# kskjs1203/SevenNet_finetuning

Measured on AMD Instinct MI355X. Metric: atoms/sec energy+force, SevenNet-0 lmax=2, 97,336-atom box @1 GPU, higher is better.
Workload: dtype f32 (MLP / linear products on bf16 MFMA pieces: bf16x6 fwd, bf16x3 bwd); 1 GPU; SevenNet-0 energy+force+virial, 97,336-atom periodic Si box (23^3 cells), 1 GPU; total_atoms=97336, scaling=weak, atoms_per_rank=97336, edges_per_rank=2725408, parallelism=single

## Files before the change

sevennet_finetuning_amd/csrc/api.cpp:

```cpp
#include <hip/hip_runtime.h>

#include <algorithm>
#include <cstdio>
#include <cstdlib>
#include <cstring>
#include <string>
#include <vector>

#include "../../include/e3gnn.h"
#include "api_util.h"
#include "atom_virial.h"
#include "cg_tables.h"
#include "common.h"
#include "dbuf.h"
#include "fused.h"
#include "generic.h"
#include "model.h"
#include "node.h"
#include "tp.h"

using namespace e3gnn;

namespace {
thread_local std::string g_err;
// ... 643 lines not shown
    const FcnDims& fd = m->fcnd;
    double flops = 2.0 * nl * dl, bytes = nl * 4.0 * (dl + 2);
    if (m->fcn) {
      double mac = fd.w[fd.nh];
      for (int k = 0; k < fd.nh; ++k) mac += (double)fd.w[k] * fd.w[k + 1];
      flops = 4.0 * nl * mac;
      bytes = nl * 4.0 * (2 * dl + 2);
    }
    Region r(c, s, C_READOUT, flops, bytes);
    if (m->fcn)
      HIPCHK(launch_readout_fcn((int)nl, fd, c->x[L].f(), m->fcn_w.f(), c->type.i(), m->scale.f(),
                                m->shift.f(), c->eat.f(), c->grad[L].f(), s));
    else
      HIPCHK(launch_readout((int)nl, dl, c->x[L].f(), m->readout_v.f(), c->type.i(), m->scale.f(),
                            m->shift.f(), c->eat.f(), s));
    HIPCHK(launch_sum(nl, c->eat.f(), c->part.f(), energy ? energy : c->scratch6.f(), s));
    if (atomic_energy && nl > 0)
      HIPCHK(hipMemcpyAsync(atomic_energy, c->eat.p, nl * 4, hipMemcpyDeviceToDevice, s));
    if (!m->fcn)
      HIPCHK(launch_readout_bwd((int)nl, dl, m->readout_v.f(), c->type.i(), m->scale.f(),
                                c->grad[L].f(), s));
  }
  c->readout_done = 1;
  return E3GNN_OK;
}

static int v1_conv_backward(e3gnn_ctx* c, int t, hipStream_t s) {
  e3gnn_model* m = c->m;
  const int64_t nl = c->nl, E = c->E;
  const int dx = irreps_dim(m->irreps[t]), dm = irreps_dim(m->mid[t]), W = m->W[t];
  const int kind = t == 0 ? 0 : (t == m->nlayer - 1 ? 2 : 1);
  {
    Region r(c, s, C_TP_BWD, 3.0 * tp_flops_per_edge(m->kcode(t)) * E,
             (double)E * 4 * (2 * W + 2 * 9 + dx + (t > 0 ? dx : 0) + 2) + nl * 4.0 * dm);
    TpArgs a;
    std::memset(&a, 0, sizeof(a));
    a.row_ptr = c->row_ptr.i();
    a.nbr = c->nbr.i();
    a.Y = c->Y.f();
    a.w = c->w[t].f();
    a.h = c->h[t].f();
    a.gagg = c->agg.f();
    a.dw = c->dw.f();
    a.dxc = t > 0 ? c->dxc.f() : nullptr;
    a.dYacc = c->dY.f();
    a.n_centers = (int)nl;
    HIPCHK(launch_tp_bwd(kind, a, s));
  }
  {
    Region r(c, s, C_MLP_BWD, 2.0 * E * (64 * W + 64 * 64 + 64 * 8),
             (double)E * 4 * (W + 64 * 6 + 16));
    auto& mm = m->mlp[t];
    GemmBatch b;
    std::memset(&b, 0, sizeof(b));
    GemmProb p = base_prob();
    p.A = c->dw.f(); p.lda = W; p.K = W;
    p.B = mm.w2t.f(); p.ldb = 64; p.N = 64;
    p.C = c->H2.f(); p.ldc = 64; p.M = (int)E;
    p.act = 2; p.pre_in = c->a2[t].f();
    add_prob(b, p);
    HIPCHK(launch_gemm(b, s));
    std::memset(&b, 0, sizeof(b));
    p.A = c->H2.f(); p.lda = 64; p.K = 64;
    p.B = mm.w1t.f(); p.C = c->H1.f(); p.pre_in = c->a1[t].f();
    add_prob(b, p);
    HIPCHK(launch_gemm(b, s));
    std::memset(&b, 0, sizeof(b));
    p.A = c->H1.f(); p.B = mm.w0t.f(); p.ldb = 8; p.N = 8;
    p.C = c->demb.f(); p.ldc = 8; p.act = 0; p.pre_in = nullptr; p.beta = 1;
    add_prob(b, p);
    HIPCHK(launch_gemm(b, s));
  }
  return E3GNN_OK;
}

int e3gnn_layer_backward_part(e3gnn_ctx* c, int t, int part, void* stream) {
  if (!c) return fail(E3GNN_ERR_ARG, "null context");
  e3gnn_model* m = c->m;
  if (t < 0 || t >= m->nlayer) return fail(E3GNN_ERR_ARG, "layer out of range");
  if (part != 0 && part != 1) return fail(E3GNN_ERR_ARG, "part must be 0 or 1");
  if (!c->readout_done) return fail(E3GNN_ERR_ARG, "e3gnn_readout must precede the backward");
  HIPCHK(hipSetDevice(m->device));
  hipStream_t s = (hipStream_t)stream;
  if (c->gen) {
    if (part == 0) HIPCHK(gen_layer_backward(c->gen, m->gen, gen_graph(c), t, s));
    return E3GNN_OK;
  }
  const int64_t n = c->n, nl = c->nl, E = c->E;
  const int dx = irreps_dim(m->irreps[t]), dg = irreps_dim(m->gin[t]);
  const int dm = irreps_dim(m->mid[t]), W = m->W[t];
  const bool last = t == m->nlayer - 1;
  const int kind = t == 0 ? 0 : (last ? 2 : 1);
  const int code = m->kcode(t);
  const int64_t n_int = c->n_int, e_int = c->e_int;
  auto out_bwd = [&]() -> int {
    {
      Region r(c, s, C_GATE_BWD, 0, nl * 4.0 * (2 * dg + irreps_dim(m->irreps[t + 1])));
      HIPCHK(launch_gate_bwd((int)nl, last, m->gdims[t], c->y[t].f(), c->grad[t + 1].f(), c->dy.f(), s));
    }
    Region r(c, s, C_LINEAR, lin_flops(*m->si2[t], nl));
    NlBatch nb;
    if (c->nodelin && nl_batch(nb, *m->nl_si2t[t], c->dy.f(), dg, nullptr, 0, c->agg.f(), dm, nl, 0))
      HIPCHK(launch_nodelin(nb, s));
    else
      HIPCHK(launch_gemm(lin_bwd(*m->si2[t], c->dy.f(), dg, c->agg.f(), dm, nl, 0), s));
    return E3GNN_OK;
  };
  auto in_bwd = [&](int64_t r0, int64_t r1, bool gather, bool owned) -> int {
    if (t == 0) return E3GNN_OK;
    if (gather && r1 > r0) {
      Region r(c, s, C_GATHER, 0, (double)E * 4 * (dx + 1) * (r1 - r0) / std::max<int64_t>(n, 1) +
                                      (r1 - r0) * 4.0 * dx);
      HIPCHK(launch_gather_rows_range((int)r0, (int)r1, dx, c->src_ptr.i(), c->src_perm.i(),
                                      c->dxc.f(), c->dh.f(), s));
    }
    Region r(c, s, C_LINEAR, lin_flops(*m->si1[t], r1 - r0) + (owned ? lin_flops(*m->sc[t], nl) : 0));
    NlBatch b0, b1;
    const int64_t p1 = owned ? nl : r0;
    if (c->nodelin && (!owned || r0 == 0) && r1 >= p1 &&
        (!owned || nl_batch(b0, *m->nl_bwd[t], c->dh.f(), dx, c->dy.f(), dg, c->grad[t].f(), dx, nl, 0)) &&
        (r1 == p1 || nl_batch(b1, *m->nl_si1t[t], c->dh.f() + p1 * dx, dx, nullptr, 0,
                              c->grad[t].f() + p1 * dx, dx, r1 - p1, 0))) {
      if (owned) HIPCHK(launch_nodelin(b0, s));
      if (r1 > p1) HIPCHK(launch_nodelin(b1, s));
    } else {
      if (r1 > r0)
        HIPCHK(launch_gemm(lin_bwd(*m->si1[t], c->dh.f() + r0 * dx, dx, c->grad[t].f() + r0 * dx, dx,
                                   r1 - r0, 0), s));
      if (owned) HIPCHK(launch_gemm(lin_bwd(*m->sc[t], c->dy.f(), dg, c->grad[t].f(), dx, nl, 1), s));
    }
    return E3GNN_OK;
  };
  if (c->graph_impl == 1) {
    if (part == 1) return E3GNN_OK;
    if (const int rc = out_bwd()) return rc;
    if (const int rc = v1_conv_backward(c, t, s)) return rc;
    return in_bwd(0, n, true, true);
  }
  if (part == 0) {
    if (const int rc = out_bwd()) return rc;
  }
  FusedArgs a = fused_base(c, t);
  a.gagg = c->agg.f();
  a.center = c->center.i();
  a.n_edges = (int)E;
  a.src_ptr = c->src_ptr.i();
  a.src_perm = c->src_perm.i();
  a.dh = c->dh.f();
  a.dxc = (!last && t > 0) ? c->dxc.f() : nullptr;
  a.dgu = c->dgu.f();
  a.demb = c->demb.f();
  a.c_begin = (int)(part == 0 ? n_int : 0);
  a.c_end = (int)(part == 0 ? nl : n_int);
  a.node_begin = (int)(part == 0 ? nl : 0);
  a.node_end = (int)(part == 0 ? n : nl);
  double ef = (double)(part == 0 ? E - e_int : e_int);
  if (last && c->timing && a.node_end > a.node_begin) {
    int32_t q[2];
    HIPCHK(hipMemcpyAsync(&q[0], a.src_ptr + a.node_begin, 4, hipMemcpyDeviceToHost, s));
    HIPCHK(hipMemcpyAsync(&q[1], a.src_ptr + a.node_end, 4, hipMemcpyDeviceToHost, s));
    HIPCHK(hipStreamSynchronize(s));
    ef = (double)(q[1] - q[0]);
  }
  if (last ? a.node_end > a.node_begin : a.c_end > a.c_begin) {
    const double xf = 3.0 * tp_flops_per_edge(code) + 2.0 * (64 * W + 64 * 64 + 8 * 64);
    Region r(c, s, C_CONV_BWD_X + kind, xf * ef,
             ef * 4 * (8 + 9 + 2 + 3 + 8) + (a.c_end - a.c_begin) * 4.0 * dm);
    HIPCHK(last ? launch_conv_bwd_nbr_last(code, a, s) : launch_conv_bwd_ls(code, a, s));
  }
  return part == 0 ? in_bwd(nl, n, !last, false) : in_bwd(0, nl, !last, true);
}

int e3gnn_layer_backward(e3gnn_ctx* c, int t, void* stream) {
  const int rc = e3gnn_layer_backward_part(c, t, 0, stream);
  return rc ? rc : e3gnn_layer_backward_part(c, t, 1, stream);
}

int e3gnn_forces(e3gnn_ctx* c, float* forces, float* virial6, float* edge_grad, void* stream) {
  if (!c) return fail(E3GNN_ERR_ARG, "null context");
  e3gnn_model* m = c->m;
  HIPCHK(hipSetDevice(m->device));
  hipStream_t s = (hipStream_t)stream;
  if (c->gen) {
    HIPCHK(gen_forces(c->gen, m->gen, gen_graph(c), forces, virial6, edge_grad, s));
    c->forces_done = 1;
    return E3GNN_OK;
  }
  const int64_t n = c->n, nl = c->nl, E = c->E;
  {
    Region r(c, s, C_EDGE_FORCE, 0, (double)E * 4 * (3 + 9 + 8 + 3));
    HIPCHK(launch_edge_force(E, c->vec.f(), m->coeffs.f(), m->cutoff, m->r_on, m->raw_sh, c->dY.f(),
                             c->dgu.f(), c->demb.f(), c->fe.f(), c->vpart.f(), s));
    HIPCHK(launch_final_sum(edge_force_blocks(E), 6, c->vpart.f(),
                            virial6 ? virial6 : c->scratch6.f(), s));
  }
  if (forces) {
    Region r(c, s, C_ATOM_FORCE, 0, (double)E * 4 * 2 * 4 + n * 12.0);
    HIPCHK(launch_atom_force((int)n, (int)nl, c->row_ptr.i(), c->src_ptr.i(), c->src_perm.i(),
                             c->fe.f(), forces, s));
  }
  if (edge_grad && E > 0)
    HIPCHK(hipMemcpyAsync(edge_grad, c->fe.p, E * 12, hipMemcpyDeviceToDevice, s));
  c->forces_done = 1;
  return E3GNN_OK;
}

int e3gnn_atom_virial(e3gnn_ctx* c, float* atom_virial6, void* stream) {
  if (!c) return fail(E3GNN_ERR_ARG, "null context");
  if (!atom_virial6) return fail(E3GNN_ERR_ARG, "null atom_virial6 output");
  if (!c->forces_done)
    return fail(E3GNN_ERR_ARG, "e3gnn_forces (or e3gnn_energy_forces) on the current graph must "
                               "precede e3gnn_atom_virial");
  HIPCHK(hipSetDevice(c->m->device));
  hipStream_t s = (hipStream_t)stream;
  const bool ordered = c->done_pending;
  if (ordered && c->done_stream != s) HIPCHK(hipStreamWaitEvent(s, c->done_ev, 0));
  const float* fe = c->gen ? gen_fe(c->gen) : c->fe.f();
  {
    Region r(c, s, C_ATOM_VIRIAL, 18.0 * 2 * c->E, (double)c->E * 4 * 2 * 7 + c->n * 24.0);
    HIPCHK(launch_atom_virial((int)c->n, (int)c->nl, c->row_ptr.i(), c->src_ptr.i(),
                              c->src_perm.i(), c->vec.f(), fe, atom_virial6, s));
  }
  if (ordered) {
    HIPCHK(hipEventRecord(c->done_ev, s));
    c->done_stream = s;
  }
  return E3GNN_OK;
}

int e3gnn_energy_forces(e3gnn_ctx* c, int64_t n_atoms, int64_t n_edges, const int32_t* type,
                        const int32_t* edge_center, const int32_t* edge_nbr,
                        const float* edge_vec, float* energy, float* atomic_energy,
                        float* forces, float* virial6, float* edge_grad, void* stream) {
  if (!energy) return fail(E3GNN_ERR_ARG, "energy output is required");
  int rc = e3gnn_graph_set(c, n_atoms, 0, n_edges, type, edge_center, edge_nbr, edge_vec, stream);
  if (rc) return rc;
  const int L = c->m->nlayer;
  for (int t = 0; t < L; ++t)
    if ((rc = e3gnn_layer_forward(c, t, stream))) return rc;
  if ((rc = e3gnn_readout(c, energy, atomic_energy, stream))) return rc;
  for (int t = L - 1; t >= 0; --t)
    if ((rc = e3gnn_layer_backward(c, t, stream))) return rc;
  if ((rc = e3gnn_forces(c, forces, virial6, edge_grad, stream))) return rc;
  if (!c->stream_ordered) {
    HIPCHK(hipStreamSynchronize((hipStream_t)stream));
  } else {
    if (!c->done_ev) HIPCHK(hipEventCreateWithFlags(&c->done_ev, hipEventDisableTiming));
    HIPCHK(hipEventRecord(c->done_ev, (hipStream_t)stream));
    c->done_stream = (hipStream_t)stream;
    c->done_pending = true;
  }
  return E3GNN_OK;
}

int e3gnn_halo_pack(const int32_t* idx, int64_t n, int dim, const float* src, int64_t src_stride,
                    float* dst, void* stream) {
  if (n < 0 || dim <= 0) return fail(E3GNN_ERR_ARG, "bad halo size");
  HIPCHK(launch_pack(n, dim, idx, src, src_stride, dst, (hipStream_t)stream));
  return E3GNN_OK;
}
int e3gnn_halo_unpack(const int32_t* idx, int64_t n, int dim, const float* src, float* dst,
                      int64_t dst_stride, int accumulate, void* stream) {
  if (n < 0 || dim <= 0) return fail(E3GNN_ERR_ARG, "bad halo size");
  HIPCHK(launch_unpack(n, dim, idx, src, dst, dst_stride, accumulate, (hipStream_t)stream));
  return E3GNN_OK;
}

int e3gnn_set_interior(e3gnn_ctx* c, int64_t n_interior) {
  if (!c) return fail(E3GNN_ERR_ARG, "null context");
  if (n_interior < 0) return fail(E3GNN_ERR_ARG, "negative n_interior");
  c->n_interior_req = n_interior;
  return E3GNN_OK;
}

int e3gnn_set_impl(e3gnn_ctx* c, int impl) {
  if (!c) return fail(E3GNN_ERR_ARG, "null context");
  if (impl != 0 && impl != 1) return fail(E3GNN_ERR_ARG, "impl must be 0 (fused) or 1 (v1)");
  c->impl = impl;
  return E3GNN_OK;
}

int e3gnn_set_timing(e3gnn_ctx* c, int enable) {
  if (!c) return fail(E3GNN_ERR_ARG, "null context");
  c->flush();
  c->timing = enable != 0;
  return E3GNN_OK;
}
int e3gnn_set_stream_ordered(e3gnn_ctx* c, int enable) {
  if (!c) return fail(E3GNN_ERR_ARG, "null context");
  c->stream_ordered = enable != 0;
  return E3GNN_OK;
}
int e3gnn_kernel_stats(e3gnn_ctx* c, const char** names, double* ms, int64_t* launches,
                       double* flops, double* bytes, int max) {
  if (!c) return -1;
  c->flush();
  for (int i = 0; i < C_NCLS && i < max; ++i) {
    if (names) names[i] = kClassNames[i];
    if (ms) ms[i] = c->stats[i].ms;
    if (launches) launches[i] = c->stats[i].launches;
    if (flops) flops[i] = c->stats[i].flops;
    if (bytes) bytes[i] = c->stats[i].bytes;
  }
  return C_NCLS;
}
int e3gnn_reset_stats(e3gnn_ctx* c) {
// ... 59 lines not shown
```

sevennet_finetuning_amd/csrc/fused.h:

```cpp
#pragma once
#include <hip/hip_runtime.h>
#include <cstdint>

namespace e3gnn {

struct MlpW {
  const float* w0;
  const float* w2r;
  const uint16_t* w2b;
  const uint16_t* w2d;
  const uint16_t* w2v;
  const uint16_t* w2s;
  const uint16_t* w1b;
  const uint16_t* w1tb;
  const uint16_t* w0tb;
};

struct FusedArgs {
  const int* row_ptr;
  const int* center;
  const int* nbr;
  const float* emb;
  const float* Y;
  const float* h;
  float* agg;
  const float* gagg;
  const int* src_ptr;
  const int* src_perm;
  float* dh;
  float* dxc;
  float* dgu;
  float* demb;
  MlpW W;
  int n_centers;
  int n_edges;
  int n_nodes;
  float denom;
  int c_begin, c_end, node_begin, node_end;
};

hipError_t launch_conv_fwd(int kind, const FusedArgs& a, hipStream_t s);
hipError_t launch_conv_bwd_ls(int kind, const FusedArgs& a, hipStream_t s);
hipError_t launch_conv_bwd_nbr_last(int kind, const FusedArgs& a, hipStream_t s);

}
```

sevennet_finetuning_amd/csrc/fused.hip:

```cpp
#include "cg_tables.h"
#include "common.h"
#include "fused.h"
#include "tp.h"
#include "w2_image.h"

#include <type_traits>


namespace e3gnn {
namespace {

typedef float f32x4 __attribute__((ext_vector_type(4)));

template <int N, int I = 0, class F>
constexpr void sfor_host(F&& f) {
  if constexpr (I < N) {
    f(std::integral_constant<int, I>{});
    sfor_host<N, I + 1>(f);
  }
}
template <int N, int I = 0, class F>
__device__ __forceinline__ void sfor(F&& f) {
  if constexpr (I < N) {
    f(std::integral_constant<int, I>{});
// ... 887 lines not shown
                wnxt[0] = w2_block_bwd<false>(hq[0], wq);
                wnxt[1] = two ? w2_block_bwd<false>(hq[1], wq) : zero4();
              }
              if (nb + 2 < NBLK) load_w2b(wq, R.w2v, lane, 16 * (nb + 2));
              float dwr2[2][4];
#pragma unroll
              for (int u = 0; u < 2; ++u) {
                if (u == 1 && !two) break;
                float dwr[4];
#pragma unroll
                for (int r = 0; r < 4; ++r) {
                  phase();
                  float dy[2 * p.l2 + 1];
#pragma unroll
                  for (int q = 0; q < 2 * p.l2 + 1; ++q) dy[q] = 0.f;
                  dwr[r] = tp_bwd_xw<p.l1, p.l2, p.l3>(x + r * D1, y[u] + yoff(p.l2), wv[u][r], gm[u] + r * D3,
                                                       dx + r * D1, dy);
                  if constexpr (p.l2 > 0) {
#pragma unroll
                    for (int q = 0; q < 2 * p.l2 + 1; ++q) dYa[u][yoff(p.l2) + q] += dy[q];
                  }
                  pin<D1>(dx + r * D1);
                  pin<8>(dYa[u] + 1);
                }
                if constexpr (NBR_DH2_BF16) {
#pragma unroll
                  for (int r = 0; r < 4; ++r) dwr2[u][r] = u == 1 && !two ? 0.f : dwr[r];
                } else {
#pragma unroll
                  for (int bh = 0; bh < 4; ++bh)
#pragma unroll
                    for (int r = 0; r < 4; ++r) dh2[u][bh] = mfma(bq[bh][r], dwr[r], dh2[u][bh]);
                }
              }
              if constexpr (NBR_DH2_BF16) {
                if (!two) {
#pragma unroll
                  for (int r = 0; r < 4; ++r) dwr2[1][r] = 0.f;
                }
                if (nb & 1) {
                  dh2_pair_g2(dh2, dwp, dwr2, two, R.w2d, nb >> 1, lane);
                } else {
#pragma unroll
                  for (int u = 0; u < 2; ++u)
#pragma unroll
                    for (int r = 0; r < 4; ++r) dwp[u][r] = dwr2[u][r];
                }
              }
              pin<4 * D1>(dx);
              wcur[0] = wnxt[0];
              wcur[1] = wnxt[1];
              ++nb;
            }
          });
          phase();
          {
            constexpr int NV = 4 * D1;
            static_assert(NV % 8 == 4, "batches of 16, 8, then 4");
            float* da = dacc + XOFF + (16 * jj + 4 * g) * D1;
            if constexpr (NV >= 16) da[own] += row_scatter16<16>(dx, rsel);
            if constexpr (NV % 16 >= 8) da[NV / 16 * 16 + (own & 7)] += row_scatter16<8>(dx + NV / 16 * 16, rsel);
            da[NV / 8 * 8 + (own & 3)] += row_scatter16<4>(dx + NV / 8 * 8, rsel);
          }
        }
      }
    });

#pragma unroll
    for (int u = 0; u < 2; ++u) {
      if (u == 1 && !two) break;
      phase();
      float d[8];
#pragma unroll
      for (int q = 0; q < 8; ++q) d[q] = sum_rows4(dYa[u][q + 1]);
      if (g == 0 && er[u] >= 0) {
        const float s3 = 1.7320508075688772f, s5 = 2.23606797749979f, c15 = s3 * s5;
        const float is3 = 0.57735026918962576f;
        const float ux = y[u][1] * is3, uy = y[u][2] * is3, uz = y[u][3] * is3;
        const float gx = s3 * d[0] + c15 * (uz * d[3] + uy * d[4]) - s5 * ux * d[5] - c15 * ux * d[7];
        const float gy = s3 * d[1] + c15 * (ux * d[4] + uz * d[6]) + 2.f * s5 * uy * d[5];
        const float gz = s3 * d[2] + c15 * (ux * d[3] + uy * d[6]) - s5 * uz * d[5] + c15 * uz * d[7];
        float* o = dgu + (int64_t)er[u] * 3;
        o[0] = gu_old[u][0] + gx;
        o[1] = gu_old[u][1] + gy;
        o[2] = gu_old[u][2] + gz;
      }
      phase();
      mlp_bwd_chain_ids(R, emb, er[u], lane, dh2[u], demb, de_old[u]);
    }
  }
  phase();
  __builtin_amdgcn_s_waitcnt(0);
  float* dhj = dh + (int64_t)jn * L::DX;
  for (int t = lane; t < L::DX; t += 64) dhj[t] = dacc[t];
}


constexpr int LS_WPC = E3GNN_BWD_W_X3 ? 2 : 3;
constexpr int LS_DPC = E3GNN_DH2_X3 ? 2 : 3;
constexpr int LS_IMG = (LS_WPC > LS_DPC ? LS_WPC : LS_DPC) * w2img::PIECE_BYTES;

template <int NPC = 3>
__device__ __forceinline__ void lds_op3(Op3& o, const char* pimg, int b, int lane) {
#pragma unroll
  for (int pc = 0; pc < NPC; ++pc)
#pragma unroll
    for (int m = 0; m < 2; ++m) o.v[pc][m] = w2img::tr_read(pimg, lane, b, pc, m);
}

__device__ __forceinline__ void dh2_pair(f32x4 (&dh2)[4], const float (&da)[4], const float (&db)[4],
                                         const char* pimg, int lane) {
  if constexpr (E3GNN_DH2_X3) {
    bf16x8 d[2];
    {
      float v[8];
#pragma unroll
      for (int t = 0; t < 8; ++t) v[t] = t < 4 ? da[t] : db[t - 4];
      split2x8(v, d);
    }
    bf16x8 a[4][2];
#pragma unroll
    for (int bh = 0; bh < 4; ++bh)
#pragma unroll
      for (int pc = 0; pc < 2; ++pc)
        a[bh][pc] = w2img::row_read(pimg, lane, pc, bh);
    phase();
#pragma unroll
    for (int bh = 0; bh < 4; ++bh) {
      dh2[bh] = mfma16(a[bh][1], d[0], dh2[bh]);
      dh2[bh] = mfma16(a[bh][0], d[1], dh2[bh]);
      dh2[bh] = mfma16(a[bh][0], d[0], dh2[bh]);
    }
    return;
  }
  bf16x8 d[3];
  {
    float v[8];
#pragma unroll
    for (int t = 0; t < 8; ++t) v[t] = t < 4 ? da[t] : db[t - 4];
    split3x8(v, d);
  }
  constexpr int I[6] = {2, 1, 0, 1, 0, 0}, J[6] = {0, 1, 2, 0, 1, 0};
#pragma unroll
  for (int bh = 0; bh < 4; ++bh) {
    bf16x8 a[3];
#pragma unroll
    for (int pc = 0; pc < 3; ++pc)
      a[pc] = w2img::row_read(pimg, lane, pc, bh);
#pragma unroll
    for (int q = 0; q < 6; ++q) dh2[bh] = mfma16(a[I[q]], d[J[q]], dh2[bh]);
  }
}

__device__ __forceinline__ int ls_tiles(const int* __restrict__ row_ptr, int cb, int c_end) {
  int T = 0;
#pragma unroll
  for (int w = 0; w < 4; ++w) {
    const int cc = cb + w;
    if (cc < c_end) T = max(T, (row_ptr[cc + 1] - row_ptr[cc] + 15) >> 4);
  }
  return __builtin_amdgcn_readfirstlane(T);
}

template <class L>
struct BwdLsWaves {
  static constexpr int v = L::KIND == 0 ? 3 : 2;
};
constexpr int LS_WPG = 4;
template <class L>
struct LsTwoImages {
  static constexpr int OFF0 = L::KIND == 1 ? L::P[0].mul : 0;
  static constexpr int DMS = L::DM - OFF0;
  static constexpr int bytes = LS_WPG * DMS * 4 + 2 * LS_IMG;
  static constexpr bool v = BwdLsWaves<L>::v * bytes <= 163840;
};
template <class L>
struct LsQuads {
  static constexpr int unroll(int npi) { return npi % 4 == 0 ? 1 : npi % 2 == 0 ? 2 : 4; }
  static constexpr bool pos_ok() {
    if (L::W / 16 % 4) return false;
    for (int i = 0; i < 3; ++i)
      if (mul_of<L>(i) > 0 && (mul_of<L>(i) / 16 % unroll(paths_of<L>(i)) || blocks_before<L>(i) % 4)) return false;
    return true;
  }
  static constexpr int bytes = LS_WPG * (L::DM - LsTwoImages<L>::OFF0) * 4 + 4 * LS_IMG;
  static constexpr bool v = L::KIND == 1 && LsTwoImages<L>::v && pos_ok() && BwdLsWaves<L>::v * bytes <= 163840;
};
template <int P>
__device__ __forceinline__ void ls_prio() { __builtin_amdgcn_s_setprio(P); }
template <class L>
__global__ __launch_bounds__(64 * LS_WPG) __attribute__((amdgpu_waves_per_eu(BwdLsWaves<L>::v, BwdLsWaves<L>::v))) void k_conv_bwd_ls(
    const int* __restrict__ row_ptr, const int* __restrict__ nbr, const float* __restrict__ emb,
    const float* __restrict__ Y, const float* __restrict__ h, const float* __restrict__ gagg, MlpW W,
    float* __restrict__ dxc, float* __restrict__ dgu, float* __restrict__ demb, int c_begin,
    int c_end, int n_nodes) {
  constexpr int NBLK = L::W / 16, NPAIR = NBLK / 2;
  static_assert(NBLK % 2 == 0, "weight blocks come in pairs");
  constexpr int WPG = LS_WPG, NT = 64 * WPG;
  constexpr int NST = LS_IMG / 16 / NT;
  static_assert(LS_IMG / 16 % NT == 0, "staging pieces per thread");
  constexpr bool TWO = LsTwoImages<L>::v;
  constexpr bool QUAD = LsQuads<L>::v;
  constexpr int NIMG = QUAD ? 2 : 1;
  constexpr bool KEEP = BwdLsWaves<L>::v == 2;
  constexpr int OFF0 = TWO ? LsTwoImages<L>::OFF0 : 0, DMS = L::DM - OFF0;
  static_assert(!TWO || (L::P[0].l1 == 0 && L::P[0].l2 == 0 && L::P[0].l3 == 0 && L::P[0].moff == 0 &&
                         OFF0 % 4 == 0), "path 0 is the 0e x 0e -> 0e slice at the row start");
  __shared__ __attribute__((aligned(16))) float smem[WPG * DMS + (TWO ? 2 : 1) * NIMG * LS_IMG / 4];
  const int tid = threadIdx.x, wid = __builtin_amdgcn_readfirstlane(tid >> 6), lane = tid & 63, g = lane >> 4, col = lane & 15;
  const int cb = c_begin + blockIdx.x * WPG;
  const int c = cb + wid;
  const bool valid = c < c_end;
  const int beg = valid ? row_ptr[c] : 0, end = valid ? row_ptr[c + 1] : 0;
  const int T = ls_tiles(row_ptr, cb, c_end);
  float* dacc = smem + wid * DMS - OFF0;
  char* img = reinterpret_cast<char*>(smem + WPG * DMS);
  if (valid && end > beg) {
    const float4* s4 = reinterpret_cast<const float4*>(gagg + (int64_t)c * L::DM + OFF0);
    float4* d4 = reinterpret_cast<float4*>(dacc + OFF0);
    for (int k = lane; k < DMS / 4; k += 64) d4[k] = s4[k];
  }
  int rb = 0;
  const __amdgpu_buffer_rsrc_t Rg0 =
      rsrc_bytes(gagg + (valid ? (int64_t)c * L::DM : 0), valid ? (int64_t)OFF0 * 4 : 0);
  const WRes R = make_wres(W, L::W);
  const __amdgpu_buffer_rsrc_t Rs = rsrc_bytes(W.w2s, NPAIR * w2img::PAIR_BYTES);
  const __amdgpu_buffer_rsrc_t Rx = rsrc_bytes(h, (int64_t)n_nodes * L::DX * 4);
  f32x4 st[NIMG * NST];
  auto issue = [&](int P) {
#pragma unroll
    for (int i = 0; i < NIMG * NST; ++i)
      st[i] = ldw4(Rs, (tid + NT * (i % NST)) * 16, (P + i / NST) * w2img::PAIR_BYTES);
  };
  auto commit = [&]() {
    __syncthreads();
#pragma unroll
    for (int i = 0; i < NST; ++i) *reinterpret_cast<f32x4*>(img + (tid + NT * i) * 16) = st[i];
    __syncthreads();
  };
  constexpr bool STAMPED = std::is_same<L, LayerMid>::value && !E3GNN_STAMPS_FWD;
  STAMP_DECL
  issue(0);
  for (int t = 0; t < T; ++t) {
    if constexpr (STAMPED) STAMP(0);
    const int q0 = beg + 16 * t;
    const bool act = q0 < end;
    const int er = (act && q0 + col < end) ? q0 + col : -1;
    const int vx = (er >= 0 ? nbr[er] : 0) * L::DX * 4;
    float xpf[20];
    float g0pf[4];
    auto load_group = [&](auto Iq, int jq) {
      constexpr int D1q = 2 * Iq + 1;
      constexpr int XOq = iblock_xoff<L, Iq>();
      ldv<4 * D1q>(Rx, vx + 4 * g * D1q * 4, (XOq + 16 * jq * D1q) * 4, xpf);
      if constexpr (OFF0 > 0 && Iq == 0) ldv<4>(Rg0, 4 * g * 4, 16 * jq * 4, g0pf);
    };
    float y[9];
    float gu_old[3] = {0.f, 0.f, 0.f}, de_old[4] = {0.f, 0.f, 0.f, 0.f};
    f32x4 a2k[4];
    float bk[2];
    Op3 hq;
    load_group(std::integral_constant<int, first_I<L>()>{}, 0);
    const int nrow = (act && dxc) ? min(16, end - q0) : 0;
    const __amdgpu_buffer_rsrc_t Rd =
        rsrc_bytes(dxc ? dxc + (int64_t)(act ? q0 : 0) * L::DX : gagg, (int64_t)nrow * L::DX * 4);
    const int vd = col * L::DX * 4;
    if (act) {
#pragma unroll
      for (int q = 0; q < 9; ++q) y[q] = er >= 0 ? Y[(int64_t)er * 9 + q] : 0.f;
      float b[2];
#pragma unroll
      for (int s = 0; s < 2; ++s) b[s] = er >= 0 ? emb[(int64_t)er * 8 + 4 * s + g] : 0.f;
      if constexpr (KEEP) {
        if (g == 0 && er >= 0) {
#pragma unroll
          for (int k = 0; k < 3; ++k) gu_old[k] = dgu[(int64_t)er * 3 + k];
        }
        if (g < 2 && er >= 0) {
#pragma unroll
          for (int k = 0; k < 4; ++k) de_old[k] = demb[(int64_t)er * 8 + 4 * g + k];
        }
      }
      MlpT m;
      mlp_chain<CX3>(R, b, lane, m);
      if constexpr (KEEP) {
#pragma unroll
        for (int bb = 0; bb < 4; ++bb) a2k[bb] = m.a2[bb];
        bk[0] = b[0];
        bk[1] = b[1];
      }
      f32x4 h2[4];
#pragma unroll
      for (int bb = 0; bb < 4; ++bb)
#pragma unroll
        for (int r = 0; r < 4; ++r) h2[bb][r] = act_fwd(m.a2[bb][r]);
      split_h2(h2, hq);
    }
    if constexpr (STAMPED) STAMP(1);
    f32x4 dh2[4] = {zero4(), zero4(), zero4(), zero4()};
    float dYa[9];
#pragma unroll
    for (int q = 0; q < 9; ++q) dYa[q] = 0.f;
    float dwp[4];
    f32x4 wv0 = zero4(), wv1 = zero4();
    sfor<3>([&](auto I) {
      constexpr int MUL = iblock_mul<L, I>();
      if constexpr (MUL > 0) {
        constexpr int D1 = 2 * I + 1;
        constexpr int XOFF = iblock_xoff<L, I>();
        constexpr int NPI = paths_of<L>(I), NB0 = blocks_before<L>(I);
        constexpr int U = QUAD ? LsQuads<L>::unroll(NPI) : (NPI & 1) ? 2 : 1;
        static_assert((MUL / 16) % U == 0, "channel groups come in pairs");
        auto groups = [&](const int j2) {
          sfor<U>([&](auto hh) {
            const int jj = j2 + hh;
            float x[4 * D1], dx[4 * D1], g0[4];
#pragma unroll
            for (int i = 0; i < 4 * D1; ++i) {
              x[i] = xpf[i];
              dx[i] = 0.f;
            }
            if constexpr (OFF0 > 0 && I == 0) {
#pragma unroll
              for (int i = 0; i < 4; ++i) g0[i] = g0pf[i];
            }
            if (jj + 1 < MUL / 16) {
              load_group(I, jj + 1);
            } else {
              constexpr int IN = next_I<L>(I);
              if constexpr (IN >= 0) load_group(std::integral_constant<int, IN>{}, 0);
            }
            sfor<L::NP>([&](auto pi) {
              constexpr PathDef p = L::P[pi];
              if constexpr (p.l1 == I) {
                constexpr int D3 = 2 * p.l3 + 1;
                constexpr int POS = (NB0 + hh * NPI + path_rank<L>(pi)) & (2 * NIMG - 1), ODD = POS & 1;
                const int nb = NB0 + jj * NPI + path_rank<L>(pi);
                const char* pimg = img + (TWO ? rb * NIMG * LS_IMG : 0) + (POS >> 1) * LS_IMG;
                if constexpr (POS == 0) {
                  if constexpr (STAMPED) STAMP(5);
                  const int nextP = (nb >> 1) + NIMG < NPAIR ? (nb >> 1) + NIMG : 0;
                  if constexpr (TWO) {
#pragma unroll
                    for (int i = 0; i < NIMG * NST; ++i)
                      *reinterpret_cast<f32x4*>(img + (rb * NIMG + i / NST) * LS_IMG + (tid + NT * (i % NST)) * 16) = st[i];
                    __syncthreads();
                    issue(nextP);
                  } else {
                    commit();
                    issue(nextP);
                  }
                  if constexpr (STAMPED) STAMP(2);
                }
                if constexpr (!ODD) {
                  if (act) {
                    ls_prio<1>();
                    Op3 wq, wq1;
                    lds_op3<LS_WPC>(wq, pimg, 0, lane);
                    lds_op3<LS_WPC>(wq1, pimg, 1, lane);
                    phase();
                    wv0 = w2_block_bwd<false>(hq, wq);
                    wv1 = w2_block_bwd<false>(hq, wq1);
                    ls_prio<0>();
                  }
                  if constexpr (STAMPED) STAMP(3);
                }
                if (act) {
                  const f32x4 wv = ODD ? wv1 : wv0;
                  float gm[4 * D3];
                  if constexpr (OFF0 > 0 && pi == 0) {
#pragma unroll
                    for (int k = 0; k < 4; ++k) gm[k] = g0[k];
                  } else {
                    const float* gl = dacc + p.moff + 16 * jj * D3 + 4 * g * D3;
#pragma unroll
                    for (int k = 0; k < 4 * D3; ++k) gm[k] = gl[k];
                  }
                  float dwr[4];
                  tp_bwd_xw4<p.l1, p.l2, p.l3>(x, y + yoff(p.l2), wv, gm, dx, dYa + yoff(p.l2), dwr);
                  if constexpr (L::KIND != 0) pin<4 * D1>(dx);
                  pin<8>(dYa + 1);
                  if constexpr (ODD) {
                    if constexpr (STAMPED) STAMP(5);
                    ls_prio<1>();
                    dh2_pair(dh2, dwp, dwr, pimg, lane);
                    ls_prio<0>();
                    if constexpr (STAMPED) STAMP(4);
                  } else {
#pragma unroll
                    for (int r = 0; r < 4; ++r) dwp[r] = dwr[r];
                  }
                }
                if constexpr (TWO && POS == 2 * NIMG - 1) rb ^= 1;
              }
            });
            if constexpr (L::KIND != 0)
              stv<4 * D1>(Rd, vd + 4 * g * D1 * 4, (XOFF + 16 * jj * D1) * 4, dx);
          });
        };
        if constexpr (QUAD) {
          sfor<MUL / 16 / U>([&](auto it) { groups(it * U); });
        } else {
          for (int j2 = 0; j2 < MUL / 16; j2 += U) groups(j2);
        }
      }
    });
    if (act) {
      {
        float d4a[4] = {dYa[1], dYa[2], dYa[3], dYa[4]}, d4b[4] = {dYa[5], dYa[6], dYa[7], dYa[8]};
        sum_rows4_n<4>(d4a);
        sum_rows4_n<4>(d4b);
#pragma unroll
        for (int q = 0; q < 4; ++q) {
          dYa[1 + q] = d4a[q];
          dYa[5 + q] = d4b[q];
        }
      }
      if (g == 0 && er >= 0) {
        const float s3 = 1.7320508075688772f, s5 = 2.23606797749979f, c15 = s3 * s5;
        const float is3 = 0.57735026918962576f;
        const float ux = y[1] * is3, uy = y[2] * is3, uz = y[3] * is3;
        const float* d = dYa + 1;
        const float gx = s3 * d[0] + c15 * (uz * d[3] + uy * d[4]) - s5 * ux * d[5] - c15 * ux * d[7];
        const float gy = s3 * d[1] + c15 * (ux * d[4] + uz * d[6]) + 2.f * s5 * uy * d[5];
        const float gz = s3 * d[2] + c15 * (ux * d[3] + uy * d[6]) - s5 * uz * d[5] + c15 * uz * d[7];
        float* o = dgu + (int64_t)er * 3;
        if constexpr (KEEP) {
          o[0] = gu_old[0] + gx;
          o[1] = gu_old[1] + gy;
          o[2] = gu_old[2] + gz;
        } else {
          o[0] += gx;
          o[1] += gy;
          o[2] += gz;
        }
      }
      if constexpr (STAMPED) STAMP(5);
      mlp_bwd_chain(R, emb, q0, end, lane, dh2, demb, KEEP ? de_old : nullptr, KEEP ? bk : nullptr,
                    KEEP ? a2k : nullptr);
    }
    if constexpr (STAMPED) STAMP(6);
  }
  if constexpr (STAMPED) STAMP_FLUSH(blockIdx.x * WPG + wid);
}

}

template <class L>
static hipError_t bwd_ls_impl(const FusedArgs& a, hipStream_t s) {
  const int nc = a.c_end - a.c_begin;
  hipLaunchKernelGGL(k_conv_bwd_ls<L>, dim3((nc + LS_WPG - 1) / LS_WPG), dim3(64 * LS_WPG), 0, s, a.row_ptr, a.nbr,
                     a.emb, a.Y, a.h, a.gagg, a.W, a.dxc, a.dgu, a.demb, a.c_begin, a.c_end, a.n_nodes);
  return hipGetLastError();
}

template <class L>
static hipError_t fwd_impl(const FusedArgs& a, hipStream_t s) {
  const int nc = a.c_end - a.c_begin;
  if (nc <= 0) return hipSuccess;
  hipLaunchKernelGGL(k_conv_fwd<L>, dim3((nc + 3) / 4), dim3(256), 0, s, a.row_ptr, a.nbr, a.emb,
                     a.Y, a.h, a.agg, a.W, a.c_begin, a.c_end, a.n_nodes, a.denom);
  return hipGetLastError();
}

template <class L>
static hipError_t bwd_nbr_impl(const FusedArgs& a, hipStream_t s) {
  const int nn = a.node_end - a.node_begin;
  hipLaunchKernelGGL(k_conv_bwd_nbr<L>, dim3((nn + 3) / 4), dim3(256), 0, s, a.src_ptr, a.src_perm,
                     a.center, a.emb, a.Y, a.h, a.gagg, a.W, a.dh, a.dgu, a.n_centers, a.node_begin,
                     a.node_end, a.demb);
  return hipGetLastError();
}

#define E3GNN_FAMILY_SWITCH(code, F_FIRST, F_MID, F_LAST)       \
  switch (code) {                                               \
    case 0: F_FIRST(0); case 1: F_MID(0); case 2: F_LAST(0);    \
    case 3: F_FIRST(1); case 4: F_MID(1); case 5: F_LAST(1);    \
    case 6: F_FIRST(2); case 7: F_MID(2); case 8: F_LAST(2);    \
    default: return hipErrorInvalidValue;                       \
  }

hipError_t launch_conv_bwd_ls(int kind, const FusedArgs& a, hipStream_t s) {
  const int nc = a.c_end - a.c_begin;
  if (nc <= 0 || a.n_nodes <= 0) return hipSuccess;
#define FIRST_(f) return bwd_ls_impl<Family<f>::First>(a, s)
#define MID_(f) return bwd_ls_impl<Family<f>::Mid>(a, s)
#define LAST_(f) return hipErrorInvalidValue
  E3GNN_FAMILY_SWITCH(kind, FIRST_, MID_, LAST_)
#undef FIRST_
#undef MID_
#undef LAST_
}

hipError_t launch_conv_fwd(int kind, const FusedArgs& a, hipStream_t s) {
#define FIRST_(f) return fwd_impl<Family<f>::First>(a, s)
#define MID_(f) return fwd_impl<Family<f>::Mid>(a, s)
#define LAST_(f) return fwd_impl<Family<f>::Last>(a, s)
  E3GNN_FAMILY_SWITCH(kind, FIRST_, MID_, LAST_)
#undef FIRST_
#undef MID_
#undef LAST_
}

hipError_t launch_conv_bwd_nbr_last(int kind, const FusedArgs& a, hipStream_t s) {
  const int nn = a.node_end - a.node_begin;
  if (nn <= 0 || a.n_nodes <= 0) return hipSuccess;
#define FIRST_(f) return hipErrorInvalidValue
#define MID_(f) return hipErrorInvalidValue
#define LAST_(f) return bwd_nbr_impl<Family<f>::Last>(a, s)
  E3GNN_FAMILY_SWITCH(kind, FIRST_, MID_, LAST_)
#undef FIRST_
#undef MID_
#undef LAST_
}

template <class L>
static void kind_dims(int* dx, int* w, int* dm) {
  *dx = L::DX;
  *w = L::W;
  *dm = L::DM;
}
bool fused_kind_dims(int code, int* dx, int* w, int* dm) {
  auto f = [&]() -> hipError_t {
#define FIRST_(f) return kind_dims<Family<f>::First>(dx, w, dm), hipSuccess
#define MID_(f) return kind_dims<Family<f>::Mid>(dx, w, dm), hipSuccess
#define LAST_(f) return kind_dims<Family<f>::Last>(dx, w, dm), hipSuccess
    E3GNN_FAMILY_SWITCH(code, FIRST_, MID_, LAST_)
#undef FIRST_
#undef MID_
#undef LAST_
  };
  return f() == hipSuccess;
}

template <class L>
constexpr double kind_tp_flops() {
  double f = 0;
  sfor_host<L::NP>([&](auto pi) {
    constexpr PathDef p = L::P[pi];
    f += (double)p.mul * (2 * CG<p.l1, p.l2, p.l3>::n + 2 * p.l3 + 1);
  });
  return f;
}
static_assert(kind_tp_flops<LayerFirst>() == 3456.0 && kind_tp_flops<LayerMid>() == 16832.0 &&
                  kind_tp_flops<LayerLast>() == 1184.0,
              "SURVEY.md 8d per-edge TP FLOP");
double fused_kind_tp_flops(int code) {
  switch (code) {
#define K_(c, f, T) \
  case c:           \
    return kind_tp_flops<Family<f>::T>();
    K_(0, 0, First) K_(1, 0, Mid) K_(2, 0, Last) K_(3, 1, First) K_(4, 1, Mid) K_(5, 1, Last)
    K_(6, 2, First) K_(7, 2, Mid) K_(8, 2, Last)
#undef K_
    default: return 0.0;
  }
}

template <class L>
static int kind_paths(PathDef* out, int max) {
  for (int p = 0; p < L::NP && p < max; ++p) out[p] = L::P[p];
  return L::NP;
}
int fused_kind_paths(int code, PathDef* out, int max) {
  auto f = [&]() -> int {
    switch (code) {
#define K_(c, f, T) \
  case c:           \
    return kind_paths<Family<f>::T>(out, max);
      K_(0, 0, First) K_(1, 0, Mid) K_(2, 0, Last) K_(3, 1, First) K_(4, 1, Mid) K_(5, 1, Last)
      K_(6, 2, First) K_(7, 2, Mid) K_(8, 2, Last)
#undef K_
      default: return 0;
    }
  };
  return f();
}

}

#ifdef E3GNN_STAMPS
extern "C" int e3gnn_debug_stamps(void* p) {
  return (int)hipMemcpyToSymbol(HIP_SYMBOL(e3gnn::g_stamp_buf), &p, sizeof(p));
}
#endif
```

Measured before the change: 2.734 million atoms/s.

## Partition edge-sorted backward kernel by edge ranges instead of per-center waves

```diff
diff --git a/sevennet_finetuning_amd/csrc/api.cpp b/sevennet_finetuning_amd/csrc/api.cpp
--- a/sevennet_finetuning_amd/csrc/api.cpp
+++ b/sevennet_finetuning_amd/csrc/api.cpp
@@ -819,6 +819,8 @@
   a.demb = c->demb.f();
   a.c_begin = (int)(part == 0 ? n_int : 0);
   a.c_end = (int)(part == 0 ? nl : n_int);
+  a.e_begin = (int)(part == 0 ? e_int : 0);
+  a.e_end = (int)(part == 0 ? E : e_int);
   a.node_begin = (int)(part == 0 ? nl : 0);
   a.node_end = (int)(part == 0 ? n : nl);
   double ef = (double)(part == 0 ? E - e_int : e_int);
diff --git a/sevennet_finetuning_amd/csrc/fused.h b/sevennet_finetuning_amd/csrc/fused.h
--- a/sevennet_finetuning_amd/csrc/fused.h
+++ b/sevennet_finetuning_amd/csrc/fused.h
@@ -37,6 +37,7 @@
   int n_nodes;
   float denom;
   int c_begin, c_end, node_begin, node_end;
+  int e_begin, e_end;
 };
 
 hipError_t launch_conv_fwd(int kind, const FusedArgs& a, hipStream_t s);
diff --git a/sevennet_finetuning_amd/csrc/fused.hip b/sevennet_finetuning_amd/csrc/fused.hip
--- a/sevennet_finetuning_amd/csrc/fused.hip
+++ b/sevennet_finetuning_amd/csrc/fused.hip
@@ -1063,15 +1063,8 @@
   }
 }
 
-__device__ __forceinline__ int ls_tiles(const int* __restrict__ row_ptr, int cb, int c_end) {
-  int T = 0;
-#pragma unroll
-  for (int w = 0; w < 4; ++w) {
-    const int cc = cb + w;
-    if (cc < c_end) T = max(T, (row_ptr[cc + 1] - row_ptr[cc] + 15) >> 4);
-  }
-  return __builtin_amdgcn_readfirstlane(T);
-}
+constexpr int LS_ROUNDS = 8;
+constexpr int ls_row_stride(int dms) { return dms + ((64 - dms * 4 % 256 + 256) % 256) / 4; }
 
 template <class L>
 struct BwdLsWaves {
@@ -1082,7 +1075,7 @@
 struct LsTwoImages {
   static constexpr int OFF0 = L::KIND == 1 ? L::P[0].mul : 0;
   static constexpr int DMS = L::DM - OFF0;
-  static constexpr int bytes = LS_WPG * DMS * 4 + 2 * LS_IMG;
+  static constexpr int bytes = LS_WPG * ls_row_stride(DMS) * 4 + 2 * LS_IMG;
   static constexpr bool v = BwdLsWaves<L>::v * bytes <= 163840;
 };
 template <class L>
@@ -1094,7 +1087,7 @@
       if (mul_of<L>(i) > 0 && (mul_of<L>(i) / 16 % unroll(paths_of<L>(i)) || blocks_before<L>(i) % 4)) return false;
     return true;
   }
-  static constexpr int bytes = LS_WPG * (L::DM - LsTwoImages<L>::OFF0) * 4 + 4 * LS_IMG;
+  static constexpr int bytes = LS_WPG * ls_row_stride(L::DM - LsTwoImages<L>::OFF0) * 4 + 4 * LS_IMG;
   static constexpr bool v = L::KIND == 1 && LsTwoImages<L>::v && pos_ok() && BwdLsWaves<L>::v * bytes <= 163840;
 };
 template <int P>
@@ -1103,8 +1096,8 @@
 __global__ __launch_bounds__(64 * LS_WPG) __attribute__((amdgpu_waves_per_eu(BwdLsWaves<L>::v, BwdLsWaves<L>::v))) void k_conv_bwd_ls(
     const int* __restrict__ row_ptr, const int* __restrict__ nbr, const float* __restrict__ emb,
     const float* __restrict__ Y, const float* __restrict__ h, const float* __restrict__ gagg, MlpW W,
-    float* __restrict__ dxc, float* __restrict__ dgu, float* __restrict__ demb, int c_begin,
-    int c_end, int n_nodes) {
+    float* __restrict__ dxc, float* __restrict__ dgu, float* __restrict__ demb,
+    const int* __restrict__ center, int e_begin, int e_end, int c_end, int n_nodes) {
   constexpr int NBLK = L::W / 16, NPAIR = NBLK / 2;
   static_assert(NBLK % 2 == 0, "weight blocks come in pairs");
   constexpr int WPG = LS_WPG, NT = 64 * WPG;
@@ -1117,23 +1110,14 @@
   constexpr int OFF0 = TWO ? LsTwoImages<L>::OFF0 : 0, DMS = L::DM - OFF0;
   static_assert(!TWO || (L::P[0].l1 == 0 && L::P[0].l2 == 0 && L::P[0].l3 == 0 && L::P[0].moff == 0 &&
                          OFF0 % 4 == 0), "path 0 is the 0e x 0e -> 0e slice at the row start");
-  __shared__ __attribute__((aligned(16))) float smem[WPG * DMS + (TWO ? 2 : 1) * NIMG * LS_IMG / 4];
+  constexpr int RS = ls_row_stride(DMS);
+  __shared__ __attribute__((aligned(16))) float smem[WPG * RS + (TWO ? 2 : 1) * NIMG * LS_IMG / 4];
   const int tid = threadIdx.x, wid = __builtin_amdgcn_readfirstlane(tid >> 6), lane = tid & 63, g = lane >> 4, col = lane & 15;
-  const int cb = c_begin + blockIdx.x * WPG;
-  const int c = cb + wid;
-  const bool valid = c < c_end;
-  const int beg = valid ? row_ptr[c] : 0, end = valid ? row_ptr[c + 1] : 0;
-  const int T = ls_tiles(row_ptr, cb, c_end);
-  float* dacc = smem + wid * DMS - OFF0;
-  char* img = reinterpret_cast<char*>(smem + WPG * DMS);
-  if (valid && end > beg) {
-    const float4* s4 = reinterpret_cast<const float4*>(gagg + (int64_t)c * L::DM + OFF0);
-    float4* d4 = reinterpret_cast<float4*>(dacc + OFF0);
-    for (int k = lane; k < DMS / 4; k += 64) d4[k] = s4[k];
-  }
+  const int ws = e_begin + blockIdx.x * (LS_ROUNDS * 16 * WPG);
+  const int we = min(ws + LS_ROUNDS * 16 * WPG, e_end);
+  char* img = reinterpret_cast<char*>(smem + WPG * RS);
+  int rhi = 0;
   int rb = 0;
-  const __amdgpu_buffer_rsrc_t Rg0 =
-      rsrc_bytes(gagg + (valid ? (int64_t)c * L::DM : 0), valid ? (int64_t)OFF0 * 4 : 0);
   const WRes R = make_wres(W, L::W);
   const __amdgpu_buffer_rsrc_t Rs = rsrc_bytes(W.w2s, NPAIR * w2img::PAIR_BYTES);
   const __amdgpu_buffer_rsrc_t Rx = rsrc_bytes(h, (int64_t)n_nodes * L::DX * 4);
@@ -1152,11 +1136,22 @@
   constexpr bool STAMPED = std::is_same<L, LayerMid>::value && !E3GNN_STAMPS_FWD;
   STAMP_DECL
   issue(0);
-  for (int t = 0; t < T; ++t) {
+  for (int qr = ws; qr < we;) {
     if constexpr (STAMPED) STAMP(0);
-    const int q0 = beg + 16 * t;
+    const int cf = __builtin_amdgcn_readfirstlane(center[qr]);
+    const int end = __builtin_amdgcn_readfirstlane(min(min(qr + 16 * WPG, we), row_ptr[min(cf + 4, c_end)]));
+    const int cl = __builtin_amdgcn_readfirstlane(center[end - 1]);
+    const int cs0 = max(cf, rhi), nnew = cl - cs0 + 1;
+    rhi = cl + 1;
+    const int q0 = qr + 16 * wid;
+    qr = end;
     const bool act = q0 < end;
     const int er = (act && q0 + col < end) ? q0 + col : -1;
+    const int dc = er >= 0 ? center[er] - cf : 0;
+    const float* dacc = smem + ((cf + dc) & 3) * RS - OFF0;
+    const __amdgpu_buffer_rsrc_t Rg0 = rsrc_bytes(
+        gagg + (int64_t)cf * L::DM, OFF0 > 0 ? ((int64_t)(cl - cf) * L::DM + OFF0) * 4 : 0);
+    const int vg0 = (dc * L::DM + 4 * g) * 4;
     const int vx = (er >= 0 ? nbr[er] : 0) * L::DX * 4;
     float xpf[20];
     float g0pf[4];
@@ -1164,7 +1159,7 @@
       constexpr int D1q = 2 * Iq + 1;
       constexpr int XOq = iblock_xoff<L, Iq>();
       ldv<4 * D1q>(Rx, vx + 4 * g * D1q * 4, (XOq + 16 * jq * D1q) * 4, xpf);
-      if constexpr (OFF0 > 0 && Iq == 0) ldv<4>(Rg0, 4 * g * 4, 16 * jq * 4, g0pf);
+      if constexpr (OFF0 > 0 && Iq == 0) ldv<4>(Rg0, vg0, 16 * jq * 4, g0pf);
     };
     float y[9];
     float gu_old[3] = {0.f, 0.f, 0.f}, de_old[4] = {0.f, 0.f, 0.f, 0.f};
@@ -1176,10 +1171,10 @@
     const __amdgpu_buffer_rsrc_t Rd =
         rsrc_bytes(dxc ? dxc + (int64_t)(act ? q0 : 0) * L::DX : gagg, (int64_t)nrow * L::DX * 4);
     const int vd = col * L::DX * 4;
+    float b[2];
     if (act) {
 #pragma unroll
       for (int q = 0; q < 9; ++q) y[q] = er >= 0 ? Y[(int64_t)er * 9 + q] : 0.f;
-      float b[2];
 #pragma unroll
       for (int s = 0; s < 2; ++s) b[s] = er >= 0 ? emb[(int64_t)er * 8 + 4 * s + g] : 0.f;
       if constexpr (KEEP) {
@@ -1192,6 +1187,24 @@
           for (int k = 0; k < 4; ++k) de_old[k] = demb[(int64_t)er * 8 + 4 * g + k];
         }
       }
+    }
+    {
+      constexpr int NRK = (DMS / 4 + NT - 1) / NT;
+      const __amdgpu_buffer_rsrc_t Rr = rsrc_bytes(
+          gagg + (int64_t)cs0 * L::DM + OFF0, nnew > 0 ? ((int64_t)(nnew - 1) * L::DM + DMS) * 4 : 0);
+      __syncthreads();
+      f32x4 rowv[4 * NRK];
+#pragma unroll
+      for (int i = 0; i < 4 * NRK; ++i)
+        rowv[i] = ldw4(Rr, ((i / NRK) * L::DM + (tid + NT * (i % NRK)) * 4) * 4, 0);
+#pragma unroll
+      for (int i = 0; i < 4 * NRK; ++i) {
+        const int k = tid + NT * (i % NRK);
+        if (i / NRK < nnew && k < DMS / 4)
+          reinterpret_cast<f32x4*>(smem + ((cs0 + i / NRK) & 3) * RS)[k] = rowv[i];
+      }
+    }
+    if (act) {
       MlpT m;
       mlp_chain<CX3>(R, b, lane, m);
       if constexpr (KEEP) {
@@ -1359,9 +1372,11 @@
 
 template <class L>
 static hipError_t bwd_ls_impl(const FusedArgs& a, hipStream_t s) {
-  const int nc = a.c_end - a.c_begin;
-  hipLaunchKernelGGL(k_conv_bwd_ls<L>, dim3((nc + LS_WPG - 1) / LS_WPG), dim3(64 * LS_WPG), 0, s, a.row_ptr, a.nbr,
-                     a.emb, a.Y, a.h, a.gagg, a.W, a.dxc, a.dgu, a.demb, a.c_begin, a.c_end, a.n_nodes);
+  const int ne = a.e_end - a.e_begin, per = LS_ROUNDS * 16 * LS_WPG;
+  if (ne <= 0) return hipSuccess;
+  hipLaunchKernelGGL(k_conv_bwd_ls<L>, dim3((ne + per - 1) / per), dim3(64 * LS_WPG), 0, s, a.row_ptr, a.nbr,
+                     a.emb, a.Y, a.h, a.gagg, a.W, a.dxc, a.dgu, a.demb, a.center, a.e_begin, a.e_end,
+                     a.c_end, a.n_nodes);
   return hipGetLastError();
 }
 
```

After: 2.847 million atoms/s (median of 6 runs). 4.1% higher.
